# kv13arm/mujoco_rl_manipulate_unknown_objects

Measured on NVIDIA B200. Metric: env-steps/sec (acorn_env, 4096 envs/GPU), higher is better.
Workload: dtype f32

## Files before the change

mujoco_rl_manipulate_unknown_objects_b200/csrc/dev_model.cpp:

```cpp
#include <cstdlib>
#include <algorithm>
#include <cstring>
#include <stdexcept>

#include "model.h"

namespace grs {

void build_dev_model(const HostModel& h, DevModel& d, std::vector<float>& hv4, std::vector<int>& adj) {
  std::memset(&d, 0, sizeof d);
  if (h.nq != NQ || h.nv != NV || h.nu != NU)
    throw std::runtime_error("scene does not have the gripper-scene shape nq=14 nv=13 nu=7 (got nq=" + std::to_string(h.nq) + " nv=" + std::to_string(h.nv) +
                             " nu=" + std::to_string(h.nu) + ")");
  if (h.nbody > MAXB || h.njnt > MAXJ || h.ngeom > MAXG || h.npair > MAXPAIR || h.ncam > MAXCAM)
    throw std::runtime_error("scene exceeds the compiled-in limits (bodies/joints/geoms/pairs/cameras)");
  if (h.body_ee < 0 || h.body_object < 0 || h.finger1[0] < 0 || h.finger1[1] < 0 || h.finger2[0] < 0 || h.finger2[1] < 0)
    throw std::runtime_error("scene lacks one of the named bodies ee / object / {left,right}_inner_{knuckle,finger}");
  d.nbody = h.nbody; d.njnt = h.njnt; d.ngeom = h.ngeom; d.npair = h.npair; d.iterations = h.iterations; d.ncam = h.ncam;
  d.timestep = (float)h.timestep; d.impratio = (float)h.impratio; d.meaninertia = (float)h.meaninertia;
  d.solver_scale = (float)(1.0 / (h.meaninertia * std::max(1, h.nv)));
  d.gap_skip = getenv("GRS_GAP_SKIP") ? atoi(getenv("GRS_GAP_SKIP")) : 1;
  d.newton_noise = getenv("GRS_NEWTON_NOISE") ? (float)atof(getenv("GRS_NEWTON_NOISE")) : 3.6e-7f;
  for (int k = 0; k < 3; k++) d.gravity[k] = (float)h.gravity[k];
  d.xfrc_ee_z = (float)(-(0.438 * h.gravity[2]));
  std::vector<int> depth(h.nbody, 0);
  int maxd = 0;
  for (int b = 1; b < h.nbody; b++) { depth[b] = depth[h.body_parentid[b]] + 1; maxd = std::max(maxd, depth[b]); }
  if (maxd + 1 > MAXLEVEL) throw std::runtime_error("kinematic tree is deeper than the compiled-in limit");
  d.nlevel = maxd + 1;
  int n = 0;
  for (int lv = 0; lv <= maxd; lv++) {
    d.level_start[lv] = n;
    for (int b = 0; b < h.nbody; b++) if (depth[b] == lv) d.level_body[n++] = b;
  }
  for (int lv = maxd + 1; lv <= MAXLEVEL; lv++) d.level_start[lv] = n;
  for (int b = 0; b < h.nbody; b++) {
    d.body_parent[b] = h.body_parentid[b]; d.body_root[b] = h.body_rootid[b];
    d.body_jntadr[b] = h.body_jntadr[b] < 0 ? 0 : h.body_jntadr[b]; d.body_jntnum[b] = h.body_jntnum[b];
    d.body_dofadr[b] = h.body_dofadr[b] < 0 ? 0 : h.body_dofadr[b]; d.body_dofnum[b] = h.body_dofnum[b];
    for (int k = 0; k < 3; k++) { d.body_pos[b][k] = (float)h.body_pos[3 * b + k]; d.body_ipos[b][k] = (float)h.body_ipos[3 * b + k]; d.body_inertia[b][k] = (float)h.body_inertia[3 * b + k]; }
    for (int k = 0; k < 4; k++) { d.body_quat[b][k] = (float)h.body_quat[4 * b + k]; d.body_iquat[b][k] = (float)h.body_iquat[4 * b + k]; }
    d.body_mass[b] = (float)h.body_mass[b];
    d.body_invweight0[b][0] = (float)h.body_invweight0[2 * b]; d.body_invweight0[b][1] = (float)h.body_invweight0[2 * b + 1];
    unsigned mask = 0;
    for (int c = 0; c < h.nbody; c++) {
      int a = c;
      while (a != b && a > 0) a = h.body_parentid[a];
      if (a == b) mask |= 1u << c;
    }
    d.body_subtree_mask[b] = mask;
    unsigned dm = 0;
    for (int a = b; a > 0; a = h.body_parentid[a])
      for (int k = 0; k < h.body_dofnum[a]; k++) dm |= 1u << (h.body_dofadr[a] + k);
    d.body_dofmask[b] = dm;
  }
  for (int j = 0; j < h.njnt; j++) {
    d.jnt_type[j] = h.jnt_type[j]; d.jnt_body[j] = h.jnt_bodyid[j]; d.jnt_qposadr[j] = h.jnt_qposadr[j];
    d.jnt_dofadr[j] = h.jnt_dofadr[j]; d.jnt_limited[j] = h.jnt_limited[j];
    for (int k = 0; k < 3; k++) { d.jnt_pos[j][k] = (float)h.jnt_pos[3 * j + k]; d.jnt_axis[j][k] = (float)h.jnt_axis[3 * j + k]; }
    d.jnt_range[j][0] = (float)h.jnt_range[2 * j]; d.jnt_range[j][1] = (float)h.jnt_range[2 * j + 1];
    d.jnt_qpos0[j] = (float)h.qpos0[h.jnt_qposadr[j]];
  }
  for (int k = 0; k < 2; k++) d.jnt_solref[k] = (float)h.jnt_solref[k];
  for (int k = 0; k < 5; k++) d.jnt_solimp[k] = (float)h.jnt_solimp[k];
  for (int k = 0; k < NQ; k++) d.qpos0[k] = (float)h.qpos0[k];
  for (int i = 0; i < NV; i++) {
    d.dof_body[i] = h.dof_bodyid[i]; d.dof_jnt[i] = h.dof_jntid[i];
    unsigned am = 0;
    for (int a = i; a >= 0; a = h.dof_parentid[a]) am |= 1u << a;
    d.dof_ancmask[i] = am;
    d.dof_armature[i] = (float)h.dof_armature[i]; d.dof_damping[i] = (float)h.dof_damping[i]; d.dof_invweight0[i] = (float)h.dof_invweight0[i];
  }
  for (int i = 0; i < NV; i++) {
    unsigned blk = i < 7 ? 0x7fu : (0x3fu << 7);
    if (d.dof_ancmask[i] & ~blk) throw std::runtime_error("dof tree layout is not 7 gripper dofs followed by 6 free-object dofs");
  }
  hv4.clear(); adj.clear();
  for (int g = 0; g < h.ngeom; g++) {
    d.geom_type[g] = h.geom_type[g]; d.geom_body[g] = h.geom_bodyid[g];
    for (int k = 0; k < 3; k++) d.geom_pos[g][k] = (float)h.geom_pos[3 * g + k];
    for (int k = 0; k < 4; k++) d.geom_quat[g][k] = (float)h.geom_quat[4 * g + k];
    d.geom_rbound[g] = (float)h.geom_rbound[g];
    for (int k = 0; k < 3; k++) d.geom_size[g][k] = (float)h.geom_size[3 * g + k];
    if (h.geom_meshid[g] >= 0) {
      const HostMesh& ms = h.meshes[h.geom_meshid[g]];
      int nvert = (int)ms.hull_verts.size() / 3;
      d.geom_hvadr[g] = (int)hv4.size() / 4; d.geom_hvnum[g] = nvert;
      for (int i = 0; i < nvert; i++) { for (int k = 0; k < 3; k++) hv4.push_back((float)ms.hull_verts[3 * i + k]); hv4.push_back(0.0f); }
      d.geom_adjadr[g] = (int)adj.size();
      adj.insert(adj.end(), ms.adjadr.begin(), ms.adjadr.end());
      adj.insert(adj.end(), ms.adj.begin(), ms.adj.end());
    }
  }
  d.nhv_total = (int)hv4.size() / 4;
  for (int p = 0; p < h.npair; p++) {
    int g1 = h.pair_geom1[p], g2 = h.pair_geom2[p];
    d.pair_g1[p] = g1; d.pair_g2[p] = g2;
    if (std::max(h.geom_condim[g1], h.geom_condim[g2]) != 4)
      throw std::runtime_error("only condim-4 contact pairs are supported (the reference scenes' default geom condim)");
    if (std::max(h.geom_gap[g1], h.geom_gap[g2]) != 0) throw std::runtime_error("geom gap is not supported");
    d.pair_margin[p] = (float)std::max(h.geom_margin[g1], h.geom_margin[g2]);
    for (int k = 0; k < 3; k++) d.pair_fric[p][k] = (float)std::max(h.geom_friction[3 * g1 + k], h.geom_friction[3 * g2 + k]);
    for (int k = 0; k < 2; k++) d.pair_solref[p][k] = (float)(0.5 * (h.geom_solref[2 * g1 + k] + h.geom_solref[2 * g2 + k]));
    for (int k = 0; k < 5; k++) d.pair_solimp[p][k] = (float)(0.5 * (h.geom_solimp[5 * g1 + k] + h.geom_solimp[5 * g2 + k]));
  }
  for (int u = 0; u < NU; u++) {
    d.act_dof[u] = h.act_dofid[u]; d.act_gear[u] = (float)h.act_gear[u];
    d.act_lo[u] = (float)std::max(-1e30, h.act_ctrlrange[2 * u]); d.act_hi[u] = (float)std::min(1e30, h.act_ctrlrange[2 * u + 1]);
  }
  d.body_ee = h.body_ee; d.body_object = h.body_object;
  for (int k = 0; k < 2; k++) { d.finger1[k] = h.finger1[k]; d.finger2[k] = h.finger2[k]; }
  for (int c = 0; c < h.ncam; c++) {
    d.cam_body[c] = h.cam_bodyid[c]; d.cam_mode[c] = h.cam_mode[c]; d.cam_target[c] = h.cam_target[c];
    for (int k = 0; k < 3; k++) d.cam_pos[c][k] = (float)h.cam_pos[3 * c + k];
    for (int k = 0; k < 4; k++) d.cam_quat[c][k] = (float)h.cam_quat[4 * c + k];
    d.cam_fovy[c] = (float)h.cam_fovy[c];
  }
}

}
```

mujoco_rl_manipulate_unknown_objects_b200/csrc/model.h:

```cpp
#pragma once
#include <array>
#include <string>
#include <vector>

namespace grs {

constexpr int NQ = 14, NV = 13, NU = 7;
constexpr int MAXB = 10, MAXJ = 8, MAXG = 8, MAXPAIR = 16, MAXMESH = 6, MAXLEVEL = 6;
constexpr int MAXCAM = 4, MAXLIGHT = 4;

enum GeomType { GEOM_PLANE = 0, GEOM_BOX = 6, GEOM_MESH = 7 };
enum JointType { JNT_FREE = 0, JNT_SLIDE = 2, JNT_HINGE = 3 };

struct HostMesh {
  std::string name;
  std::array<double, 3> pos{};
  std::array<double, 4> quat{1, 0, 0, 0};
  double volume = 0;
  std::array<double, 3> inertia_unit{};
  std::vector<double> hull_verts;
  std::vector<int> hull_faces;
  std::vector<int> adjadr, adj;
  std::vector<float> tri;
};

struct HostModel {
  int nbody = 0, njnt = 0, nq = 0, nv = 0, nu = 0, ngeom = 0, nmesh = 0, npair = 0, ncam = 0, nlight = 0;
  double timestep = 0.002, gravity[3] = {0, 0, -9.81}, impratio = 1, tolerance = 1e-8, znear = 0.01, zfar = 50;
  int iterations = 100, cone_elliptic = 0;
  std::vector<std::string> body_names, geom_names, jnt_names, cam_names;
  std::vector<int> body_parentid, body_weldid, body_jntadr, body_jntnum, body_dofadr, body_dofnum, body_rootid;
  std::vector<double> body_pos, body_quat, body_ipos, body_iquat, body_mass, body_inertia, body_invweight0;
  std::vector<int> jnt_type, jnt_bodyid, jnt_qposadr, jnt_dofadr, jnt_limited;
  std::vector<double> jnt_pos, jnt_axis, jnt_range, qpos0;
  double jnt_solref[2] = {0.02, 1}, jnt_solimp[5] = {0.9, 0.95, 0.001, 0.5, 2};
  std::vector<int> dof_bodyid, dof_jntid, dof_parentid;
  std::vector<double> dof_armature, dof_damping, dof_invweight0;
  std::vector<int> geom_type, geom_bodyid, geom_meshid, geom_condim;
  std::vector<double> geom_pos, geom_quat, geom_friction, geom_margin, geom_gap, geom_solref, geom_solimp,
      geom_rbound, geom_rgba, geom_size, geom_mass, geom_matprop;
  std::vector<HostMesh> meshes;
  std::vector<int> act_dofid;
  std::vector<double> act_gear, act_ctrlrange;
  std::vector<int> pair_geom1, pair_geom2;
  std::vector<int> cam_bodyid, cam_mode, cam_target;
  std::vector<double> cam_pos, cam_quat, cam_fovy;
  std::vector<int> light_bodyid, light_directional;
  std::vector<double> light_pos, light_dir, light_diffuse, light_ambient, light_specular;
  double meaninertia = 1, extent = 1, center[3] = {0, 0, 0};
  double tex_rgb1[3] = {0.1, 0.2, 0.3}, tex_rgb2[3] = {0.2, 0.3, 0.4}, texrepeat[2] = {1, 1};
  double sky_rgb1[3] = {0.3, 0.5, 0.7}, sky_rgb2[3] = {0, 0, 0};
  int body_ee = -1, body_object = -1, finger1[2] = {-1, -1}, finger2[2] = {-1, -1};
};

HostModel compile_mjcf(const std::string& xml_path);

struct DevModel {
  int nbody, njnt, ngeom, npair, nlevel, nhv_total, iterations, ncam;
  float timestep, impratio, meaninertia, solver_scale;
  int gap_skip;
  float newton_noise;
  float gravity[3], xfrc_ee_z;
  int level_start[MAXLEVEL + 1];
  int level_body[MAXB];
  int body_parent[MAXB], body_root[MAXB], body_jntadr[MAXB], body_jntnum[MAXB], body_dofadr[MAXB], body_dofnum[MAXB];
  unsigned body_subtree_mask[MAXB];
  unsigned body_dofmask[MAXB];
  float body_pos[MAXB][3], body_quat[MAXB][4], body_ipos[MAXB][3], body_iquat[MAXB][4];
  float body_mass[MAXB], body_inertia[MAXB][3], body_invweight0[MAXB][2];
  int jnt_type[MAXJ], jnt_body[MAXJ], jnt_qposadr[MAXJ], jnt_dofadr[MAXJ], jnt_limited[MAXJ];
  float jnt_pos[MAXJ][3], jnt_axis[MAXJ][3], jnt_range[MAXJ][2], jnt_qpos0[MAXJ];
  float jnt_solref[2], jnt_solimp[5], padj;
  float qpos0[NQ + 2];
  int dof_body[NV + 3], dof_jnt[NV + 3];
  unsigned dof_ancmask[NV + 3];
  float dof_armature[NV + 3], dof_damping[NV + 3], dof_invweight0[NV + 3];
  int geom_type[MAXG], geom_body[MAXG], geom_hvadr[MAXG], geom_hvnum[MAXG], geom_adjadr[MAXG];
  float geom_pos[MAXG][3], geom_quat[MAXG][4], geom_rbound[MAXG], geom_size[MAXG][3];
  int pair_g1[MAXPAIR], pair_g2[MAXPAIR];
  float pair_margin[MAXPAIR], pair_fric[MAXPAIR][3] , pair_solref[MAXPAIR][2], pair_solimp[MAXPAIR][5];
  int act_dof[NU + 1];
  float act_gear[NU + 1], act_lo[NU + 1], act_hi[NU + 1];
  int body_ee, body_object, finger1[2], finger2[2], pad2, pad3;
  int cam_body[MAXCAM], cam_mode[MAXCAM], cam_target[MAXCAM];
  float cam_pos[MAXCAM][3], cam_quat[MAXCAM][4], cam_fovy[MAXCAM];
};

void build_dev_model(const HostModel& h, DevModel& d, std::vector<float>& hull_verts4, std::vector<int>& hull_adj);

}
```

mujoco_rl_manipulate_unknown_objects_b200/csrc/sim_kernels.cuh:

```cuda
#pragma once
#include <cuda_runtime.h>
#include <stdint.h>

#include "model.h"

namespace grs {

constexpr int MAXCON = 12;
constexpr int MAXEFC = MAXCON * 4 + 7;
constexpr unsigned FULL = 0xffffffffu;
constexpr float MINVAL = 1e-15f;

struct __align__(16) WS {
  float qpos[16], qvel[16], ctrl[8], warm[16];
  float xpos[MAXB][3], xquat[MAXB][4], xmat[MAXB][9];
  float xanchor[MAXJ][3], xaxis[MAXJ][3];
  float gpos[MAXG][3], gmat[MAXG][9];
  float com[MAXB][3];
  float cdof[16][6];
  float M[NV * NV];
  int ncon, nefc, nlim, overflow, coupled, padi[3];
  float c_dist[MAXCON], c_pos[MAXCON][3], c_frame[MAXCON][9], c_mu[MAXCON], c_fric[MAXCON][3];
  int c_g1[MAXCON], c_g2[MAXCON], c_pair[MAXCON];
  float fsmooth[16], asmooth[16], qacc[16], Ma[16], grad[16], search[16], Mv[16], fcon[16], bias[16];
// ... 110 lines not shown
  for (int k = 0; k < NB; k++) {
    a[k] = 0.0f;
    if (k < nb) {
      if (is_row && k <= lr) a[k] = A[lane * NV + base + k];
      else if (is_rhs) a[k] = tmp[base + k];
    }
  }
#pragma unroll
  for (int j = 0; j < NB; j++) {
    if (is_row && lr >= j) A[lane * NV + base + j] = a[j];
    __syncwarp();
    const int cj = base + (j < nb ? j : 0);
    const float djj = A[cj * NV + cj];
    float rs = rsqrtf(fmaxf(djj, 1e-30f));
    rs = rs * (1.5f - 0.5f * djj * rs * rs);
    const float t = a[j] * rs * rs;
    a[j] *= rs;
#pragma unroll
    for (int k = j + 1; k < NB; k++) {
      const int rk = base + (k < nb ? k : 0);
      a[k] -= t * A[rk * NV + cj];
    }
  }
  __syncwarp();
  if (is_row) {
#pragma unroll
    for (int k = 0; k < NB; k++)
      if (k <= lr) A[lane * NV + base + k] = a[k];
  }
  if (is_rhs) {
#pragma unroll
    for (int k = 0; k < NB; k++)
      if (k < nb) tmp[base + k] = a[k];
  }
  __syncwarp();
  float y = is_row ? tmp[lane] : 0.0f;
#pragma unroll
  for (int j = NB - 1; j >= 0; j--) {
    const bool valid = j < nb;
    const int gj = base + (valid ? j : 0);
    const float ljj = A[gj * NV + gj];
    if (is_row && valid && lr == j) tmp[gj] = __fdividef(y, ljj);
    __syncwarp();
    const float xj = tmp[gj];
    if (is_row && valid) {
      if (lr == j) y = xj;
      else if (lr < j) y -= A[gj * NV + lane] * xj;
    }
  }
  __syncwarp();
  return y;
}

__device__ __noinline__ void kinematics(const DevModel& m, WS& w, int lane) {
  if (lane == 0) {
    for (int j = 0; j < m.njnt; j++)
      if (m.jnt_type[j] == JNT_FREE) quat_normalize(w.qpos + m.jnt_qposadr[j] + 3);
    w.xpos[0][0] = w.xpos[0][1] = w.xpos[0][2] = 0;
    w.xquat[0][0] = 1; w.xquat[0][1] = w.xquat[0][2] = w.xquat[0][3] = 0;
    quat2mat(w.xmat[0], w.xquat[0]);
  }
  __syncwarp();
  for (int lv = 1; lv < m.nlevel; lv++) {
    int idx = m.level_start[lv] + lane;
    if (idx < m.level_start[lv + 1]) {
      int b = m.level_body[idx], pid = m.body_parent[b];
      int jadr = m.body_jntadr[b], jnum = m.body_jntnum[b];
      float pos[3], quat[4];
      if (jnum == 1 && m.jnt_type[jadr] == JNT_FREE) {
        int qa = m.jnt_qposadr[jadr];
        for (int k = 0; k < 3; k++) pos[k] = w.qpos[qa + k];
        for (int k = 0; k < 4; k++) quat[k] = w.qpos[qa + 3 + k];
        for (int k = 0; k < 3; k++) { w.xanchor[jadr][k] = pos[k]; w.xaxis[jadr][k] = 0; }
      } else {
        float t[3];
        mulmat3vec(t, w.xmat[pid], m.body_pos[b]);
        for (int k = 0; k < 3; k++) pos[k] = w.xpos[pid][k] + t[k];
        quat_mul(quat, w.xquat[pid], m.body_quat[b]);
        for (int kj = 0; kj < jnum; kj++) {
          int j = jadr + kj;
          float anchor[3], axis[3];
          rot_vec_quat(t, m.jnt_pos[j], quat);
          for (int k = 0; k < 3; k++) anchor[k] = pos[k] + t[k];
          rot_vec_quat(axis, m.jnt_axis[j], quat);
          float q = w.qpos[m.jnt_qposadr[j]] - m.jnt_qpos0[j];
          if (m.jnt_type[j] == JNT_SLIDE) {
            for (int k = 0; k < 3; k++) pos[k] += axis[k] * q;
          } else {
            float s, c, ql[4];
            sincosf(0.5f * q, &s, &c);
            ql[0] = c; ql[1] = m.jnt_axis[j][0] * s; ql[2] = m.jnt_axis[j][1] * s; ql[3] = m.jnt_axis[j][2] * s;
            quat_mul(quat, quat, ql);
            rot_vec_quat(t, m.jnt_pos[j], quat);
            for (int k = 0; k < 3; k++) pos[k] = anchor[k] - t[k];
          }
          for (int k = 0; k < 3; k++) { w.xanchor[j][k] = anchor[k]; w.xaxis[j][k] = axis[k]; }
        }
      }
      quat_normalize(quat);
      for (int k = 0; k < 3; k++) w.xpos[b][k] = pos[k];
      for (int k = 0; k < 4; k++) w.xquat[b][k] = quat[k];
      quat2mat(w.xmat[b], quat);
    }
    __syncwarp();
  }
  if (lane < m.ngeom) {
    int g = lane, b = m.geom_body[g];
    float t[3], q[4], R[9];
    mulmat3vec(t, w.xmat[b], m.geom_pos[g]);
    quat_mul(q, w.xquat[b], m.geom_quat[g]);
    quat_normalize(q);
    quat2mat(R, q);
    float d2 = 0, r2 = 0;
    for (int k = 0; k < 3; k++) { const float np_ = w.xpos[b][k] + t[k], d = np_ - w.gpos[g][k]; d2 += d * d; w.gpos[g][k] = np_; }
    for (int k = 0; k < 9; k++) { const float d = R[k] - w.gmat[g][k]; r2 += d * d; w.gmat[g][k] = R[k]; }
    w.disp[g] = sqrtf(d2) + m.geom_rbound[g] * sqrtf(r2);
  }
  __syncwarp();
}

__device__ __noinline__ void com_pos_crb(const DevModel& m, WS& w, int lane) {
  const int nb = m.nbody;
  if (lane < nb) {
    int b = lane;
    float t[3], qi[4];
    mulmat3vec(t, w.xmat[b], m.body_ipos[b]);
    for (int k = 0; k < 3; k++) w.u.dyn.xipos[b][k] = w.xpos[b][k] + t[k];
    quat_mul(qi, w.xquat[b], m.body_iquat[b]);
    quat2mat(w.u.dyn.ximat[b], qi);
  }
  __syncwarp();
  if (lane < nb) {
    int r = m.body_root[lane];
    unsigned mask = m.body_subtree_mask[r];
    float s[3] = {0, 0, 0}, ms = 0;
    for (int b = 1; b < nb; b++)
      if ((mask >> b) & 1u) {
        float mb = m.body_mass[b];
        ms += mb;
        for (int k = 0; k < 3; k++) s[k] += mb * w.u.dyn.xipos[b][k];
      }
    if (ms < MINVAL) { for (int k = 0; k < 3; k++) w.com[lane][k] = w.u.dyn.xipos[r][k]; }
    else { float inv = 1.0f / ms; for (int k = 0; k < 3; k++) w.com[lane][k] = s[k] * inv; }
  }
  __syncwarp();
  if (lane < nb) {
    int b = lane;
    float* c = w.u.dyn.cinert[b];
    if (b == 0) { for (int k = 0; k < 10; k++) c[k] = 0; }
    else {
      const float* R = w.u.dyn.ximat[b];
      const float* I = m.body_inertia[b];
      float mb = m.body_mass[b], off[3];
      for (int k = 0; k < 3; k++) off[k] = w.u.dyn.xipos[b][k] - w.com[b][k];
      float dd = dot3(off, off);
      float M00 = R[0] * I[0] * R[0] + R[1] * I[1] * R[1] + R[2] * I[2] * R[2];
      float M11 = R[3] * I[0] * R[3] + R[4] * I[1] * R[4] + R[5] * I[2] * R[5];
      float M22 = R[6] * I[0] * R[6] + R[7] * I[1] * R[7] + R[8] * I[2] * R[8];
      float M01 = R[0] * I[0] * R[3] + R[1] * I[1] * R[4] + R[2] * I[2] * R[5];
      float M02 = R[0] * I[0] * R[6] + R[1] * I[1] * R[7] + R[2] * I[2] * R[8];
      float M12 = R[3] * I[0] * R[6] + R[4] * I[1] * R[7] + R[5] * I[2] * R[8];
      c[0] = M00 + mb * (dd - off[0] * off[0]);
      c[1] = M11 + mb * (dd - off[1] * off[1]);
      c[2] = M22 + mb * (dd - off[2] * off[2]);
      c[3] = M01 - mb * off[0] * off[1];
      c[4] = M02 - mb * off[0] * off[2];
      c[5] = M12 - mb * off[1] * off[2];
      c[6] = mb * off[0]; c[7] = mb * off[1]; c[8] = mb * off[2];
      c[9] = mb;
    }
  }
  if (lane < NV) {
    int i = lane, j = m.dof_jnt[i], b = m.dof_body[i], da = m.jnt_dofadr[j];
    float* c = w.cdof[i];
    int type = m.jnt_type[j];
    if (type == JNT_FREE) {
      int k = i - da;
      if (k < 3) { c[0] = c[1] = c[2] = 0; c[3] = k == 0; c[4] = k == 1; c[5] = k == 2; }
      else {
        k -= 3;
        float ax[3] = {w.xmat[b][k], w.xmat[b][3 + k], w.xmat[b][6 + k]}, off[3];
        for (int q = 0; q < 3; q++) off[q] = w.com[b][q] - w.xpos[b][q];
        c[0] = ax[0]; c[1] = ax[1]; c[2] = ax[2];
        cross3(c + 3, ax, off);
      }
    } else if (type == JNT_SLIDE) {
      c[0] = c[1] = c[2] = 0;
      for (int q = 0; q < 3; q++) c[3 + q] = w.xaxis[j][q];
    } else {
      float off[3], ax[3];
      for (int q = 0; q < 3; q++) { off[q] = w.com[b][q] - w.xanchor[j][q]; ax[q] = w.xaxis[j][q]; c[q] = ax[q]; }
      cross3(c + 3, ax, off);
    }
  }
  __syncwarp();
  if (lane < nb) {
    int b = lane;
    unsigned mask = m.body_subtree_mask[b];
    float acc[10];
    for (int k = 0; k < 10; k++) acc[k] = 0;
    if (b > 0)
      for (int bb = b; bb < nb; bb++)
        if ((mask >> bb) & 1u)
          for (int k = 0; k < 10; k++) acc[k] += w.u.dyn.cinert[bb][k];
    for (int k = 0; k < 10; k++) w.u.dyn.crb[b][k] = acc[k];
  }
  __syncwarp();
  float buf[6];
  if (lane < NV) mul_inert_vec(buf, w.u.dyn.crb[m.dof_body[lane]], w.cdof[lane]);
  float(*fb)[6] = w.u.dyn.cdofdot;
  if (lane < NV) for (int k = 0; k < 6; k++) fb[lane][k] = buf[k];
  __syncwarp();
  for (int e = lane; e < NV * NV; e += 32) {
    int i = e / NV, j = e - i * NV;
    int hi = i > j ? i : j, lo = i > j ? j : i;
    float v = 0;
    if ((m.dof_ancmask[hi] >> lo) & 1u) v = dot6(w.cdof[lo], fb[hi]);
    if (i == j) v += m.dof_armature[i];
    w.M[e] = v;
  }
  __syncwarp();
}

#define SUPV(k) (w.sup[k])
#define SUPV1(k) (w.sup[k] + 3)
#define SUPV2(k) (w.sup[k] + 6)

__device__ __forceinline__ unsigned sortable_key(float x) {
  const unsigned k = __float_as_uint(x + 0.0f);
  return (k & 0x80000000u) ? ~k : (k | 0x80000000u);
}
__device__ __noinline__ int support_geom(const DevModel& m, const WS& w, const float4* __restrict__ hv, int g, const float* dir, float* out, int lane) {
  const float* R = w.gmat[g];
  float l[3];
  mulmat3Tvec(l, R, dir);
  const float4* v = hv + m.geom_hvadr[g];
  const int n = m.geom_hvnum[g];
  float best = -3.0e38f;
  int bi = 0;
#pragma unroll 2
  for (int i = lane; i < n; i += 32) {
    float4 p = v[i];
    float s = fmaf(p.z, l[2], fmaf(p.y, l[1], p.x * l[0]));
    if (s > best) { best = s; bi = i; }
  }
  const unsigned key = sortable_key(best);
  const unsigned kmax = __reduce_max_sync(FULL, key);
  bi = (int)__reduce_min_sync(FULL, key == kmax ? (unsigned)bi : 0xffffffffu);
  float4 p = v[bi];
  float pv[3] = {p.x, p.y, p.z}, t[3];
  mulmat3vec(t, R, pv);
  out[0] = w.gpos[g][0] + t[0]; out[1] = w.gpos[g][1] + t[1]; out[2] = w.gpos[g][2] + t[2];
  return bi;
}
__device__ __noinline__ void support_md(const DevModel& m, WS& w, const float4* hv, int g1, int g2, float margin, const float* dir, int slot, int lane) {
  float n[3] = {dir[0], dir[1], dir[2]}, nd[3];
  normalize3(n);
  nd[0] = -n[0]; nd[1] = -n[1]; nd[2] = -n[2];
  const float *R1 = w.gmat[g1], *R2 = w.gmat[g2];
  float l1[3], l2[3];
  mulmat3Tvec(l1, R1, n);
  mulmat3Tvec(l2, R2, nd);
  const float4 *va = hv + m.geom_hvadr[g1], *vb = hv + m.geom_hvadr[g2];
  const int na = m.geom_hvnum[g1], nb = m.geom_hvnum[g2], nmax = max(na, nb);
  float besta = -3.0e38f, bestb = -3.0e38f;
  int ia = 0, ib = 0;
#pragma unroll 2
  for (int i = lane; i < nmax; i += 32) {
    if (i < na) {
      const float4 p = va[i];
// ... 244 lines not shown
      for (int k = 0; k < 3; k++) dif[k] = v[k] - w.gpos[g1][k];
      float dist = dot3(dif, n);
      if (dist > margin) continue;
      for (int k = 0; k < 3; k++) pos[k] = v[k] - 0.5f * dist * n[k];
      add_contact(m, w, p, dist, pos, n, lane);
      const int* ga = adj + m.geom_adjadr[g2];
      int nvert = m.geom_hvnum[g2];
      int e0 = __ldg(ga + vi), e1 = __ldg(ga + vi + 1), cnt = 1;
      const float4* hvg = hv + m.geom_hvadr[g2];
      for (int e = e0; e < e1 && cnt < 3; e++) {
        int nb = __ldg(ga + nvert + 1 + e);
        float4 q = hvg[nb];
        float qv[3] = {q.x, q.y, q.z}, t[3];
        mulmat3vec(t, w.gmat[g2], qv);
        for (int k = 0; k < 3; k++) { v[k] = w.gpos[g2][k] + t[k]; dif[k] = v[k] - w.gpos[g1][k]; }
        dist = dot3(dif, n);
        if (dist > margin) continue;
        for (int k = 0; k < 3; k++) pos[k] = v[k] - 0.5f * dist * n[k];
        add_contact(m, w, p, dist, pos, n, lane);
        cnt++;
      }
    } else {
      float depth, dir[3], pos[3];
      float ca[3] = {w.sep[p][0], w.sep[p][1], w.sep[p][2]};
      if (ca[0] != 0.0f || ca[1] != 0.0f || ca[2] != 0.0f) {
        support_md(m, w, hv, g1, g2, margin, ca, 4, lane);
        const float sd = dot3(SUPV(4), ca);
        if (sd < 0) {
          __syncwarp();
          if (lane == 0) w.gapb[p] = -sd - 2e-6f;
          __syncwarp();
          continue;
        }
      }
      bool hit = mpr_penetration(m, w, hv, g1, g2, margin, &depth, dir, pos, lane);
      __syncwarp();
      if (lane < 3) w.sep[p][lane] = hit ? 0.0f : dir[lane];
      if (lane == 3) w.gapb[p] = 0.0f;
      __syncwarp();
      if (!hit) continue;
      add_contact(m, w, p, margin - depth, pos, dir, lane);
    }
  }
  __syncwarp();
}

__device__ __forceinline__ void forward_position(const DevModel& m, WS& w, const float4* hv, const int* adj, int lane) {
  kinematics(m, w, lane);
  com_pos_crb(m, w, lane);
  collision(m, w, hv, adj, lane);
}

__device__ __noinline__ void smooth_forces(const DevModel& m, WS& w, int lane, bool actuation, float xfrc_z) {
  const int nb = m.nbody;
  if (lane == 0) for (int k = 0; k < 6; k++) { w.u.dyn.cvel[0][k] = 0; w.u.dyn.cfrc[0][k] = 0; }
  if (lane == 0) { float* a = w.u.dyn.crb[0]; a[0] = a[1] = a[2] = 0; a[3] = -m.gravity[0]; a[4] = -m.gravity[1]; a[5] = -m.gravity[2]; }
  __syncwarp();
  for (int lv = 1; lv < m.nlevel; lv++) {
    int idx = m.level_start[lv] + lane;
    if (idx < m.level_start[lv + 1]) {
      int b = m.level_body[idx], pid = m.body_parent[b];
      float cvel[6], cacc[6];
      for (int k = 0; k < 6; k++) { cvel[k] = w.u.dyn.cvel[pid][k]; cacc[k] = w.u.dyn.crb[pid][k]; }
      for (int kj = 0; kj < m.body_jntnum[b]; kj++) {
        int j = m.body_jntadr[b] + kj, a = m.jnt_dofadr[j];
        if (m.jnt_type[j] == JNT_FREE) {
          for (int i = 0; i < 3; i++) {
            for (int k = 0; k < 6; k++) w.u.dyn.cdofdot[a + i][k] = 0;
            float qv = w.qvel[a + i];
            for (int k = 0; k < 6; k++) cvel[k] += w.cdof[a + i][k] * qv;
          }
          float dd[3][6];
          for (int i = 0; i < 3; i++) cross_motion(dd[i], cvel, w.cdof[a + 3 + i]);
          for (int i = 0; i < 3; i++) {
            float qv = w.qvel[a + 3 + i];
            for (int k = 0; k < 6; k++) { w.u.dyn.cdofdot[a + 3 + i][k] = dd[i][k]; cvel[k] += w.cdof[a + 3 + i][k] * qv; cacc[k] += dd[i][k] * qv; }
          }
        } else {
          float dd[6], qv = w.qvel[a];
          cross_motion(dd, cvel, w.cdof[a]);
          for (int k = 0; k < 6; k++) { w.u.dyn.cdofdot[a][k] = dd[k]; cvel[k] += w.cdof[a][k] * qv; cacc[k] += dd[k] * qv; }
        }
      }
      float t1[6], t2[6], f[6];
      mul_inert_vec(t1, w.u.dyn.cinert[b], cacc);
      mul_inert_vec(t2, w.u.dyn.cinert[b], cvel);
      cross_force(f, cvel, t2);
      for (int k = 0; k < 6; k++) { w.u.dyn.cvel[b][k] = cvel[k]; w.u.dyn.crb[b][k] = cacc[k]; w.u.dyn.cfrc[b][k] = f[k] + t1[k]; }
    }
    __syncwarp();
  }
  float bias = 0;
  if (lane < NV) {
    int b = m.dof_body[lane];
    unsigned mask = m.body_subtree_mask[b];
    float acc[6] = {0, 0, 0, 0, 0, 0};
    for (int bb = b; bb < nb; bb++)
      if ((mask >> bb) & 1u)
        for (int k = 0; k < 6; k++) acc[k] += w.u.dyn.cfrc[bb][k];
    bias = dot6(w.cdof[lane], acc);
  }
  float f = 0;
  if (lane < NV) {
    f = -m.dof_damping[lane] * w.qvel[lane] - bias;
    if (actuation)
      for (int u = 0; u < NU; u++)
        if (m.act_dof[u] == lane) f += m.act_gear[u] * fminf(fmaxf(w.ctrl[u], m.act_lo[u]), m.act_hi[u]);
    if (xfrc_z != 0.0f && ((m.body_dofmask[m.body_ee] >> lane) & 1u)) {
      float off[3], t[3];
      for (int k = 0; k < 3; k++) off[k] = w.u.dyn.xipos[m.body_ee][k] - w.com[m.body_ee][k];
      cross3(t, w.cdof[lane], off);
      f += (w.cdof[lane][5] + t[2]) * xfrc_z;
    }
    w.bias[lane] = bias;
    w.fsmooth[lane] = f;
  }
  __syncwarp();
  for (int e = lane; e < NV * NV; e += 32) w.u.dyn.L[e] = w.M[e];
  __syncwarp();
  float a = chol_factor_solve<true>(w.u.dyn.L, w.cho, f, lane);
  if (lane < NV) w.asmooth[lane] = a;
  __syncwarp();
}

__device__ __noinline__ float get_impedance(const float* solimp, float pos, float margin) {
  if (solimp[0] == solimp[1] || solimp[2] <= MINVAL) return 0.5f * (solimp[0] + solimp[1]);
  float x = fabsf((pos - margin) / solimp[2]);
  if (x >= 1) return solimp[1];
  if (x <= 0) return solimp[0];
  float y, p = solimp[4], mid = solimp[3];
  if (p == 1.0f) y = x;
  else if (p == 2.0f) y = x <= mid ? x * x / mid : 1 - (1 - x) * (1 - x) / (1 - mid);
  else y = x <= mid ? powf(x, p) / powf(mid, p - 1) : 1 - powf(1 - x, p) / powf(1 - mid, p - 1);
  return solimp[0] + y * (solimp[1] - solimp[0]);
}

__device__ __noinline__ void make_constraint(const DevModel& m, WS& w, int lane) {
  bool active = false;
  float dist = 0, sign = 0;
  if (lane < m.njnt && m.jnt_limited[lane] && m.jnt_type[lane] != JNT_FREE) {
    float value = w.qpos[m.jnt_qposadr[lane]];
    float dl = value - m.jnt_range[lane][0], du = m.jnt_range[lane][1] - value;
    if (dl < 0) { active = true; dist = dl; sign = 1; }
    else if (du < 0) { active = true; dist = du; sign = -1; }
  }
  unsigned bal = __ballot_sync(FULL, active);
  int nlim = __popc(bal);
  int ncon = w.ncon;
  int nefc = nlim + 4 * ncon;
  for (int e = lane; e < nefc * NV; e += 32) (&w.u.con.J[0][0])[e] = 0;
// ... 365 lines not shown
```

Before: 24.88 million.

## Specialize kinematic tree traversal to compile-time gripper topology

Replaces the runtime level tables, subtree masks, dof ancestry masks and joint-type dispatch with compile-time constants for the fixed gripper tree, checked on the host and by static asserts. Kinematics, CRB and smooth-force passes now unroll over known bodies and joints. Hinge sin/cos values are computed in parallel across lanes before the level loop instead of serially inside it. The aim is fewer model-memory loads, fewer branches and less serial latency, at the cost of rejecting any scene with a different topology.

```diff
diff --git a/mujoco_rl_manipulate_unknown_objects_b200/csrc/dev_model.cpp b/mujoco_rl_manipulate_unknown_objects_b200/csrc/dev_model.cpp
--- a/mujoco_rl_manipulate_unknown_objects_b200/csrc/dev_model.cpp
+++ b/mujoco_rl_manipulate_unknown_objects_b200/csrc/dev_model.cpp
@@ -6,6 +6,22 @@
 #include "model.h"
 
 namespace grs {
+
+static void check_tree(const HostModel& h) {
+  auto same = [](const std::vector<int>& v, const int* t, int n) { return (int)v.size() == n && std::equal(v.begin(), v.end(), t); };
+  const char* what = nullptr;
+  if (h.nbody != tree::NBODY || h.njnt != tree::NJNT) what = "body / joint count";
+  else if (!same(h.body_parentid, tree::body_parent, tree::NBODY)) what = "body_parentid";
+  else if (!same(h.body_rootid, tree::body_root, tree::NBODY)) what = "body_rootid";
+  else if (!same(h.body_jntadr, tree::body_jntadr, tree::NBODY) || !same(h.body_jntnum, tree::body_jntnum, tree::NBODY)) what = "body_jntadr / body_jntnum";
+  else if (!same(h.body_dofadr, tree::body_dofadr, tree::NBODY) || !same(h.body_dofnum, tree::body_dofnum, tree::NBODY)) what = "body_dofadr / body_dofnum";
+  else if (!same(h.jnt_type, tree::jnt_type, tree::NJNT) || !same(h.jnt_bodyid, tree::jnt_body, tree::NJNT)) what = "joint types / joint bodies";
+  else if (!same(h.jnt_qposadr, tree::jnt_qposadr, tree::NJNT) || !same(h.jnt_dofadr, tree::jnt_dofadr, tree::NJNT)) what = "jnt_qposadr / jnt_dofadr";
+  else if (!same(h.dof_bodyid, tree::dof_body, NV) || !same(h.dof_parentid, tree::dof_parent, NV)) what = "dof_bodyid / dof_parentid";
+  if (what)
+    throw std::runtime_error(std::string("scene's kinematic tree differs from the gripper tree the step kernel is written for (") + what +
+                             "): world, two camera mounts, ee with 3 slides + 2 hinges, base link, two hinged knuckles with a finger each, one free object");
+}
 
 void build_dev_model(const HostModel& h, DevModel& d, std::vector<float>& hv4, std::vector<int>& adj) {
   std::memset(&d, 0, sizeof d);
@@ -16,6 +32,7 @@
     throw std::runtime_error("scene exceeds the compiled-in limits (bodies/joints/geoms/pairs/cameras)");
   if (h.body_ee < 0 || h.body_object < 0 || h.finger1[0] < 0 || h.finger1[1] < 0 || h.finger2[0] < 0 || h.finger2[1] < 0)
     throw std::runtime_error("scene lacks one of the named bodies ee / object / {left,right}_inner_{knuckle,finger}");
+  check_tree(h);
   d.nbody = h.nbody; d.njnt = h.njnt; d.ngeom = h.ngeom; d.npair = h.npair; d.iterations = h.iterations; d.ncam = h.ncam;
   d.timestep = (float)h.timestep; d.impratio = (float)h.impratio; d.meaninertia = (float)h.meaninertia;
   d.solver_scale = (float)(1.0 / (h.meaninertia * std::max(1, h.nv)));
@@ -23,32 +40,13 @@
   d.newton_noise = getenv("GRS_NEWTON_NOISE") ? (float)atof(getenv("GRS_NEWTON_NOISE")) : 3.6e-7f;
   for (int k = 0; k < 3; k++) d.gravity[k] = (float)h.gravity[k];
   d.xfrc_ee_z = (float)(-(0.438 * h.gravity[2]));
-  std::vector<int> depth(h.nbody, 0);
-  int maxd = 0;
-  for (int b = 1; b < h.nbody; b++) { depth[b] = depth[h.body_parentid[b]] + 1; maxd = std::max(maxd, depth[b]); }
-  if (maxd + 1 > MAXLEVEL) throw std::runtime_error("kinematic tree is deeper than the compiled-in limit");
-  d.nlevel = maxd + 1;
-  int n = 0;
-  for (int lv = 0; lv <= maxd; lv++) {
-    d.level_start[lv] = n;
-    for (int b = 0; b < h.nbody; b++) if (depth[b] == lv) d.level_body[n++] = b;
-  }
-  for (int lv = maxd + 1; lv <= MAXLEVEL; lv++) d.level_start[lv] = n;
   for (int b = 0; b < h.nbody; b++) {
-    d.body_parent[b] = h.body_parentid[b]; d.body_root[b] = h.body_rootid[b];
-    d.body_jntadr[b] = h.body_jntadr[b] < 0 ? 0 : h.body_jntadr[b]; d.body_jntnum[b] = h.body_jntnum[b];
-    d.body_dofadr[b] = h.body_dofadr[b] < 0 ? 0 : h.body_dofadr[b]; d.body_dofnum[b] = h.body_dofnum[b];
+    d.body_root[b] = h.body_rootid[b];
+    d.body_jntadr[b] = h.body_jntadr[b] < 0 ? 0 : h.body_jntadr[b];
     for (int k = 0; k < 3; k++) { d.body_pos[b][k] = (float)h.body_pos[3 * b + k]; d.body_ipos[b][k] = (float)h.body_ipos[3 * b + k]; d.body_inertia[b][k] = (float)h.body_inertia[3 * b + k]; }
     for (int k = 0; k < 4; k++) { d.body_quat[b][k] = (float)h.body_quat[4 * b + k]; d.body_iquat[b][k] = (float)h.body_iquat[4 * b + k]; }
     d.body_mass[b] = (float)h.body_mass[b];
     d.body_invweight0[b][0] = (float)h.body_invweight0[2 * b]; d.body_invweight0[b][1] = (float)h.body_invweight0[2 * b + 1];
-    unsigned mask = 0;
-    for (int c = 0; c < h.nbody; c++) {
-      int a = c;
-      while (a != b && a > 0) a = h.body_parentid[a];
-      if (a == b) mask |= 1u << c;
-    }
-    d.body_subtree_mask[b] = mask;
     unsigned dm = 0;
     for (int a = b; a > 0; a = h.body_parentid[a])
       for (int k = 0; k < h.body_dofnum[a]; k++) dm |= 1u << (h.body_dofadr[a] + k);
@@ -65,15 +63,7 @@
   for (int k = 0; k < 5; k++) d.jnt_solimp[k] = (float)h.jnt_solimp[k];
   for (int k = 0; k < NQ; k++) d.qpos0[k] = (float)h.qpos0[k];
   for (int i = 0; i < NV; i++) {
-    d.dof_body[i] = h.dof_bodyid[i]; d.dof_jnt[i] = h.dof_jntid[i];
-    unsigned am = 0;
-    for (int a = i; a >= 0; a = h.dof_parentid[a]) am |= 1u << a;
-    d.dof_ancmask[i] = am;
     d.dof_armature[i] = (float)h.dof_armature[i]; d.dof_damping[i] = (float)h.dof_damping[i]; d.dof_invweight0[i] = (float)h.dof_invweight0[i];
-  }
-  for (int i = 0; i < NV; i++) {
-    unsigned blk = i < 7 ? 0x7fu : (0x3fu << 7);
-    if (d.dof_ancmask[i] & ~blk) throw std::runtime_error("dof tree layout is not 7 gripper dofs followed by 6 free-object dofs");
   }
   hv4.clear(); adj.clear();
   for (int g = 0; g < h.ngeom; g++) {
diff --git a/mujoco_rl_manipulate_unknown_objects_b200/csrc/model.h b/mujoco_rl_manipulate_unknown_objects_b200/csrc/model.h
--- a/mujoco_rl_manipulate_unknown_objects_b200/csrc/model.h
+++ b/mujoco_rl_manipulate_unknown_objects_b200/csrc/model.h
@@ -6,11 +6,42 @@
 namespace grs {
 
 constexpr int NQ = 14, NV = 13, NU = 7;
-constexpr int MAXB = 10, MAXJ = 8, MAXG = 8, MAXPAIR = 16, MAXMESH = 6, MAXLEVEL = 6;
+constexpr int MAXB = 10, MAXJ = 8, MAXG = 8, MAXPAIR = 16, MAXMESH = 6;
 constexpr int MAXCAM = 4, MAXLIGHT = 4;
 
 enum GeomType { GEOM_PLANE = 0, GEOM_BOX = 6, GEOM_MESH = 7 };
 enum JointType { JNT_FREE = 0, JNT_SLIDE = 2, JNT_HINGE = 3 };
+
+namespace tree {
+enum Body { WORLD = 0, CAM0 = 1, CAM1 = 2, EE = 3, BASE = 4, LKNUCKLE = 5, LFINGER = 6, RKNUCKLE = 7, RFINGER = 8, OBJECT = 9, NBODY = 10 };
+constexpr int NJNT = 8, JOBJECT = 7;
+constexpr int body_parent[NBODY] = {0, WORLD, WORLD, WORLD, EE, BASE, LKNUCKLE, BASE, RKNUCKLE, WORLD};
+constexpr int body_root[NBODY] = {WORLD, CAM0, CAM1, EE, EE, EE, EE, EE, EE, OBJECT};
+constexpr int body_jntadr[NBODY] = {-1, -1, -1, 0, -1, 5, -1, 6, -1, JOBJECT};
+constexpr int body_jntnum[NBODY] = {0, 0, 0, 5, 0, 1, 0, 1, 0, 1};
+constexpr int body_dofadr[NBODY] = {-1, -1, -1, 0, -1, 5, -1, 6, -1, 7};
+constexpr int body_dofnum[NBODY] = {0, 0, 0, 5, 0, 1, 0, 1, 0, 6};
+constexpr int jnt_type[NJNT] = {JNT_SLIDE, JNT_SLIDE, JNT_SLIDE, JNT_HINGE, JNT_HINGE, JNT_HINGE, JNT_HINGE, JNT_FREE};
+constexpr int jnt_body[NJNT] = {EE, EE, EE, EE, EE, LKNUCKLE, RKNUCKLE, OBJECT};
+constexpr int jnt_qposadr[NJNT] = {0, 1, 2, 3, 4, 5, 6, 7};
+constexpr int jnt_dofadr[NJNT] = {0, 1, 2, 3, 4, 5, 6, 7};
+constexpr int dof_body[NV] = {EE, EE, EE, EE, EE, LKNUCKLE, RKNUCKLE, OBJECT, OBJECT, OBJECT, OBJECT, OBJECT, OBJECT};
+constexpr int dof_parent[NV] = {-1, 0, 1, 2, 3, 4, 4, -1, 7, 8, 9, 10, 11};
+constexpr unsigned subtree_mask(int b) {
+  unsigned mask = 0;
+  for (int c = 0; c < NBODY; c++) {
+    int a = c;
+    while (a != b && a > 0) a = body_parent[a];
+    if (a == b) mask |= 1u << c;
+  }
+  return mask;
+}
+constexpr bool dof_is_ancestor(int hi, int lo) {
+  for (int a = hi; a >= 0; a = dof_parent[a])
+    if (a == lo) return true;
+  return false;
+}
+}
 
 struct HostMesh {
   std::string name;
@@ -56,15 +87,12 @@
 HostModel compile_mjcf(const std::string& xml_path);
 
 struct DevModel {
-  int nbody, njnt, ngeom, npair, nlevel, nhv_total, iterations, ncam;
+  int nbody, njnt, ngeom, npair, nhv_total, iterations, ncam;
   float timestep, impratio, meaninertia, solver_scale;
   int gap_skip;
   float newton_noise;
   float gravity[3], xfrc_ee_z;
-  int level_start[MAXLEVEL + 1];
-  int level_body[MAXB];
-  int body_parent[MAXB], body_root[MAXB], body_jntadr[MAXB], body_jntnum[MAXB], body_dofadr[MAXB], body_dofnum[MAXB];
-  unsigned body_subtree_mask[MAXB];
+  int body_root[MAXB], body_jntadr[MAXB];
   unsigned body_dofmask[MAXB];
   float body_pos[MAXB][3], body_quat[MAXB][4], body_ipos[MAXB][3], body_iquat[MAXB][4];
   float body_mass[MAXB], body_inertia[MAXB][3], body_invweight0[MAXB][2];
@@ -72,8 +100,6 @@
   float jnt_pos[MAXJ][3], jnt_axis[MAXJ][3], jnt_range[MAXJ][2], jnt_qpos0[MAXJ];
   float jnt_solref[2], jnt_solimp[5], padj;
   float qpos0[NQ + 2];
-  int dof_body[NV + 3], dof_jnt[NV + 3];
-  unsigned dof_ancmask[NV + 3];
   float dof_armature[NV + 3], dof_damping[NV + 3], dof_invweight0[NV + 3];
   int geom_type[MAXG], geom_body[MAXG], geom_hvadr[MAXG], geom_hvnum[MAXG], geom_adjadr[MAXG];
   float geom_pos[MAXG][3], geom_quat[MAXG][4], geom_rbound[MAXG], geom_size[MAXG][3];
diff --git a/mujoco_rl_manipulate_unknown_objects_b200/csrc/sim_kernels.cuh b/mujoco_rl_manipulate_unknown_objects_b200/csrc/sim_kernels.cuh
--- a/mujoco_rl_manipulate_unknown_objects_b200/csrc/sim_kernels.cuh
+++ b/mujoco_rl_manipulate_unknown_objects_b200/csrc/sim_kernels.cuh
@@ -186,49 +186,109 @@
   return y;
 }
 
+static_assert(tree::jnt_qposadr[tree::JOBJECT] == 7 && tree::jnt_dofadr[tree::JOBJECT] == 7, "free joint at qpos 7 / dof 7");
+static_assert(tree::jnt_qposadr[6] == 6 && tree::jnt_dofadr[6] == 6, "hinges and slides: qpos address = dof address = joint id");
+static_assert(tree::jnt_type[0] == JNT_SLIDE && tree::jnt_type[1] == JNT_SLIDE && tree::jnt_type[2] == JNT_SLIDE && tree::jnt_type[3] == JNT_HINGE && tree::jnt_type[4] == JNT_HINGE && tree::jnt_type[5] == JNT_HINGE &&
+              tree::jnt_type[6] == JNT_HINGE, "joint types as kinematics writes them out");
+
+constexpr unsigned long long pack_subtrees(int first, int n) {
+  unsigned long long p = 0;
+  for (int i = 0; i < n; i++) p |= (unsigned long long)tree::subtree_mask(first + i) << (10 * i);
+  return p;
+}
+constexpr unsigned long long SUBTREE_LO = pack_subtrees(0, 6), SUBTREE_HI = pack_subtrees(6, tree::NBODY - 6);
+__host__ __device__ constexpr unsigned subtree_of(int b) {
+  return (unsigned)((b < 6 ? SUBTREE_LO >> (10 * b) : SUBTREE_HI >> (10 * (b - 6))) & 0x3ffu);
+}
+struct DepthSlot { int b, pid; bool on; };
+__host__ __device__ constexpr DepthSlot depth_slot(int d, int lane) {
+  return d == 1 ? DepthSlot{lane < 3 ? lane + 1 : tree::OBJECT, tree::WORLD, lane < 4}
+       : d == 2 ? DepthSlot{tree::BASE, tree::EE, lane == 0}
+       : DepthSlot{(d == 3 ? tree::LKNUCKLE : tree::LFINGER) + 2 * lane, d == 3 ? tree::BASE : tree::LFINGER + 2 * lane - 1, lane < 2};
+}
+constexpr int NDEPTH = 4;
+__host__ __device__ constexpr int jnt_first(int b) { return b == tree::EE ? 0 : b == tree::LKNUCKLE ? 5 : 6; }
+__host__ __device__ constexpr int jnt_count(int b) { return b == tree::EE ? 5 : b == tree::LKNUCKLE || b == tree::RKNUCKLE ? 1 : 0; }
+__host__ __device__ constexpr int root_of(int b) { return b < tree::EE ? b : b < tree::OBJECT ? tree::EE : tree::OBJECT; }
+__host__ __device__ constexpr int dof_body_of(int i) { return i < 5 ? tree::EE : i == 5 ? tree::LKNUCKLE : i == 6 ? tree::RKNUCKLE : tree::OBJECT; }
+__host__ __device__ constexpr bool dof_anc(int hi, int lo) { return hi < 7 ? (lo <= 4 || lo == hi) : lo >= 7; }
+constexpr bool lane_maps_match_tree() {
+  for (int b = 0; b < tree::NBODY; b++)
+    if (subtree_of(b) != tree::subtree_mask(b) || (subtree_of(b) & ((1u << b) - 1u)) || root_of(b) != tree::body_root[b]) return false;
+  int depth[tree::NBODY] = {0};
+  for (int d = 1; d <= NDEPTH; d++)
+    for (int lane = 0; lane < 32; lane++) {
+      const DepthSlot t = depth_slot(d, lane);
+      if (!t.on) continue;
+      if (depth[t.b] || t.pid != tree::body_parent[t.b] || depth[t.pid] != d - 1) return false;
+      depth[t.b] = d;
+      if (t.b != tree::OBJECT && (jnt_count(t.b) != tree::body_jntnum[t.b] || (jnt_count(t.b) && jnt_first(t.b) != tree::body_jntadr[t.b]))) return false;
+    }
+  for (int b = 1; b < tree::NBODY; b++)
+    if (!depth[b]) return false;
+  for (int i = 0; i < NV; i++) {
+    if (dof_body_of(i) != tree::dof_body[i]) return false;
+    for (int j = 0; j <= i; j++)
+      if (dof_anc(i, j) != tree::dof_is_ancestor(i, j)) return false;
+  }
+  return true;
+}
+static_assert(lane_maps_match_tree(), "lane maps disagree with the tree tables of model.h");
+
 __device__ __noinline__ void kinematics(const DevModel& m, WS& w, int lane) {
+  using namespace tree;
+  constexpr int QF = jnt_qposadr[JOBJECT];
   if (lane == 0) {
-    for (int j = 0; j < m.njnt; j++)
-      if (m.jnt_type[j] == JNT_FREE) quat_normalize(w.qpos + m.jnt_qposadr[j] + 3);
+    quat_normalize(w.qpos + QF + 3);
     w.xpos[0][0] = w.xpos[0][1] = w.xpos[0][2] = 0;
     w.xquat[0][0] = 1; w.xquat[0][1] = w.xquat[0][2] = w.xquat[0][3] = 0;
     quat2mat(w.xmat[0], w.xquat[0]);
   }
-  __syncwarp();
-  for (int lv = 1; lv < m.nlevel; lv++) {
-    int idx = m.level_start[lv] + lane;
-    if (idx < m.level_start[lv + 1]) {
-      int b = m.level_body[idx], pid = m.body_parent[b];
-      int jadr = m.body_jntadr[b], jnum = m.body_jntnum[b];
+  float* hsc = &w.u.dyn.cfrc[0][0];
+  if (lane >= 3 && lane < 7) {
+    float s, c;
+    sincosf(0.5f * (w.qpos[lane] - m.jnt_qpos0[lane]), &s, &c);
+    hsc[2 * (lane - 3)] = s; hsc[2 * (lane - 3) + 1] = c;
+  }
+  __syncwarp();
+#pragma unroll 1
+  for (int d = 1; d <= NDEPTH; d++) {
+    const DepthSlot t = depth_slot(d, lane);
+    if (t.on) {
+      const int b = t.b, pid = t.pid;
       float pos[3], quat[4];
-      if (jnum == 1 && m.jnt_type[jadr] == JNT_FREE) {
-        int qa = m.jnt_qposadr[jadr];
-        for (int k = 0; k < 3; k++) pos[k] = w.qpos[qa + k];
-        for (int k = 0; k < 4; k++) quat[k] = w.qpos[qa + 3 + k];
-        for (int k = 0; k < 3; k++) { w.xanchor[jadr][k] = pos[k]; w.xaxis[jadr][k] = 0; }
+      if (b == OBJECT) {
+        for (int k = 0; k < 3; k++) pos[k] = w.qpos[QF + k];
+        for (int k = 0; k < 4; k++) quat[k] = w.qpos[QF + 3 + k];
+        for (int k = 0; k < 3; k++) { w.xanchor[JOBJECT][k] = pos[k]; w.xaxis[JOBJECT][k] = 0; }
       } else {
         float t[3];
         mulmat3vec(t, w.xmat[pid], m.body_pos[b]);
         for (int k = 0; k < 3; k++) pos[k] = w.xpos[pid][k] + t[k];
         quat_mul(quat, w.xquat[pid], m.body_quat[b]);
-        for (int kj = 0; kj < jnum; kj++) {
-          int j = jadr + kj;
+        auto joint = [&](int j, bool slide) {
           float anchor[3], axis[3];
           rot_vec_quat(t, m.jnt_pos[j], quat);
           for (int k = 0; k < 3; k++) anchor[k] = pos[k] + t[k];
           rot_vec_quat(axis, m.jnt_axis[j], quat);
-          float q = w.qpos[m.jnt_qposadr[j]] - m.jnt_qpos0[j];
-          if (m.jnt_type[j] == JNT_SLIDE) {
+          float q = w.qpos[j] - m.jnt_qpos0[j];
+          if (slide) {
             for (int k = 0; k < 3; k++) pos[k] += axis[k] * q;
           } else {
-            float s, c, ql[4];
-            sincosf(0.5f * q, &s, &c);
+            const float s = hsc[2 * (j - 3)], c = hsc[2 * (j - 3) + 1];
+            float ql[4];
             ql[0] = c; ql[1] = m.jnt_axis[j][0] * s; ql[2] = m.jnt_axis[j][1] * s; ql[3] = m.jnt_axis[j][2] * s;
             quat_mul(quat, quat, ql);
             rot_vec_quat(t, m.jnt_pos[j], quat);
             for (int k = 0; k < 3; k++) pos[k] = anchor[k] - t[k];
           }
           for (int k = 0; k < 3; k++) { w.xanchor[j][k] = anchor[k]; w.xaxis[j][k] = axis[k]; }
+        };
+        if (b == EE) {
+#pragma unroll
+          for (int j = 0; j < 5; j++) joint(j, j < 3);
+        } else if (jnt_count(b)) {
+          joint(jnt_first(b), false);
         }
       }
       quat_normalize(quat);
@@ -254,8 +314,8 @@
 }
 
 __device__ __noinline__ void com_pos_crb(const DevModel& m, WS& w, int lane) {
-  const int nb = m.nbody;
-  if (lane < nb) {
+  using namespace tree;
+  if (lane < NBODY) {
     int b = lane;
     float t[3], qi[4];
     mulmat3vec(t, w.xmat[b], m.body_ipos[b]);
@@ -264,11 +324,12 @@
     quat2mat(w.u.dyn.ximat[b], qi);
   }
   __syncwarp();
-  if (lane < nb) {
-    int r = m.body_root[lane];
-    unsigned mask = m.body_subtree_mask[r];
+  if (lane < NBODY) {
+    const int r = root_of(lane);
+    const unsigned mask = subtree_of(r);
     float s[3] = {0, 0, 0}, ms = 0;
-    for (int b = 1; b < nb; b++)
+#pragma unroll
+    for (int b = 1; b < NBODY; b++)
       if ((mask >> b) & 1u) {
         float mb = m.body_mass[b];
         ms += mb;
@@ -278,7 +339,7 @@
     else { float inv = 1.0f / ms; for (int k = 0; k < 3; k++) w.com[lane][k] = s[k] * inv; }
   }
   __syncwarp();
-  if (lane < nb) {
+  if (lane < NBODY) {
     int b = lane;
     float* c = w.u.dyn.cinert[b];
     if (b == 0) { for (int k = 0; k < 10; k++) c[k] = 0; }
@@ -305,51 +366,54 @@
     }
   }
   if (lane < NV) {
-    int i = lane, j = m.dof_jnt[i], b = m.dof_body[i], da = m.jnt_dofadr[j];
+    const int i = lane;
     float* c = w.cdof[i];
-    int type = m.jnt_type[j];
-    if (type == JNT_FREE) {
-      int k = i - da;
+    if (i >= 7) {
+      int k = i - 7;
       if (k < 3) { c[0] = c[1] = c[2] = 0; c[3] = k == 0; c[4] = k == 1; c[5] = k == 2; }
       else {
         k -= 3;
-        float ax[3] = {w.xmat[b][k], w.xmat[b][3 + k], w.xmat[b][6 + k]}, off[3];
-        for (int q = 0; q < 3; q++) off[q] = w.com[b][q] - w.xpos[b][q];
+        float ax[3] = {w.xmat[OBJECT][k], w.xmat[OBJECT][3 + k], w.xmat[OBJECT][6 + k]}, off[3];
+        for (int q = 0; q < 3; q++) off[q] = w.com[OBJECT][q] - w.xpos[OBJECT][q];
         c[0] = ax[0]; c[1] = ax[1]; c[2] = ax[2];
         cross3(c + 3, ax, off);
       }
-    } else if (type == JNT_SLIDE) {
+    } else if (i < 3) {
       c[0] = c[1] = c[2] = 0;
-      for (int q = 0; q < 3; q++) c[3 + q] = w.xaxis[j][q];
+      for (int q = 0; q < 3; q++) c[3 + q] = w.xaxis[i][q];
     } else {
+      const int b = dof_body_of(i);
       float off[3], ax[3];
-      for (int q = 0; q < 3; q++) { off[q] = w.com[b][q] - w.xanchor[j][q]; ax[q] = w.xaxis[j][q]; c[q] = ax[q]; }
+      for (int q = 0; q < 3; q++) { off[q] = w.com[b][q] - w.xanchor[i][q]; ax[q] = w.xaxis[i][q]; c[q] = ax[q]; }
       cross3(c + 3, ax, off);
     }
   }
   __syncwarp();
-  if (lane < nb) {
+  if (lane < NBODY) {
     int b = lane;
-    unsigned mask = m.body_subtree_mask[b];
+    const unsigned mask = b > 0 ? subtree_of(b) : 0u;
     float acc[10];
     for (int k = 0; k < 10; k++) acc[k] = 0;
-    if (b > 0)
-      for (int bb = b; bb < nb; bb++)
-        if ((mask >> bb) & 1u)
-          for (int k = 0; k < 10; k++) acc[k] += w.u.dyn.cinert[bb][k];
+#pragma unroll
+    for (int bb = 1; bb < NBODY; bb++)
+      if ((mask >> bb) & 1u)
+        for (int k = 0; k < 10; k++) acc[k] += w.u.dyn.cinert[bb][k];
     for (int k = 0; k < 10; k++) w.u.dyn.crb[b][k] = acc[k];
   }
   __syncwarp();
   float buf[6];
-  if (lane < NV) mul_inert_vec(buf, w.u.dyn.crb[m.dof_body[lane]], w.cdof[lane]);
+  if (lane < NV) mul_inert_vec(buf, w.u.dyn.crb[dof_body_of(lane)], w.cdof[lane]);
   float(*fb)[6] = w.u.dyn.cdofdot;
   if (lane < NV) for (int k = 0; k < 6; k++) fb[lane][k] = buf[k];
   __syncwarp();
-  for (int e = lane; e < NV * NV; e += 32) {
+#pragma unroll
+  for (int it = 0; it < (NV * NV + 31) / 32; it++) {
+    const int e = lane + 32 * it;
+    if (e >= NV * NV) break;
     int i = e / NV, j = e - i * NV;
     int hi = i > j ? i : j, lo = i > j ? j : i;
     float v = 0;
-    if ((m.dof_ancmask[hi] >> lo) & 1u) v = dot6(w.cdof[lo], fb[hi]);
+    if (dof_anc(hi, lo)) v = dot6(w.cdof[lo], fb[hi]);
     if (i == j) v += m.dof_armature[i];
     w.M[e] = v;
   }
@@ -700,34 +764,41 @@
 }
 
 __device__ __noinline__ void smooth_forces(const DevModel& m, WS& w, int lane, bool actuation, float xfrc_z) {
-  const int nb = m.nbody;
+  using namespace tree;
   if (lane == 0) for (int k = 0; k < 6; k++) { w.u.dyn.cvel[0][k] = 0; w.u.dyn.cfrc[0][k] = 0; }
   if (lane == 0) { float* a = w.u.dyn.crb[0]; a[0] = a[1] = a[2] = 0; a[3] = -m.gravity[0]; a[4] = -m.gravity[1]; a[5] = -m.gravity[2]; }
   __syncwarp();
-  for (int lv = 1; lv < m.nlevel; lv++) {
-    int idx = m.level_start[lv] + lane;
-    if (idx < m.level_start[lv + 1]) {
-      int b = m.level_body[idx], pid = m.body_parent[b];
+#pragma unroll 1
+  for (int d = 1; d <= NDEPTH; d++) {
+    const DepthSlot t = depth_slot(d, lane);
+    if (t.on) {
+      const int b = t.b, pid = t.pid;
       float cvel[6], cacc[6];
       for (int k = 0; k < 6; k++) { cvel[k] = w.u.dyn.cvel[pid][k]; cacc[k] = w.u.dyn.crb[pid][k]; }
-      for (int kj = 0; kj < m.body_jntnum[b]; kj++) {
-        int j = m.body_jntadr[b] + kj, a = m.jnt_dofadr[j];
-        if (m.jnt_type[j] == JNT_FREE) {
-          for (int i = 0; i < 3; i++) {
-            for (int k = 0; k < 6; k++) w.u.dyn.cdofdot[a + i][k] = 0;
-            float qv = w.qvel[a + i];
-            for (int k = 0; k < 6; k++) cvel[k] += w.cdof[a + i][k] * qv;
-          }
-          float dd[3][6];
-          for (int i = 0; i < 3; i++) cross_motion(dd[i], cvel, w.cdof[a + 3 + i]);
-          for (int i = 0; i < 3; i++) {
-            float qv = w.qvel[a + 3 + i];
-            for (int k = 0; k < 6; k++) { w.u.dyn.cdofdot[a + 3 + i][k] = dd[i][k]; cvel[k] += w.cdof[a + 3 + i][k] * qv; cacc[k] += dd[i][k] * qv; }
-          }
-        } else {
+      if (b == OBJECT) {
+        constexpr int a = jnt_dofadr[JOBJECT];
+        for (int i = 0; i < 3; i++) {
+          for (int k = 0; k < 6; k++) w.u.dyn.cdofdot[a + i][k] = 0;
+          float qv = w.qvel[a + i];
+          for (int k = 0; k < 6; k++) cvel[k] += w.cdof[a + i][k] * qv;
+        }
+        float dd[3][6];
+        for (int i = 0; i < 3; i++) cross_motion(dd[i], cvel, w.cdof[a + 3 + i]);
+        for (int i = 0; i < 3; i++) {
+          float qv = w.qvel[a + 3 + i];
+          for (int k = 0; k < 6; k++) { w.u.dyn.cdofdot[a + 3 + i][k] = dd[i][k]; cvel[k] += w.cdof[a + 3 + i][k] * qv; cacc[k] += dd[i][k] * qv; }
+        }
+      } else {
+        auto dof = [&](int a) {
           float dd[6], qv = w.qvel[a];
           cross_motion(dd, cvel, w.cdof[a]);
           for (int k = 0; k < 6; k++) { w.u.dyn.cdofdot[a][k] = dd[k]; cvel[k] += w.cdof[a][k] * qv; cacc[k] += dd[k] * qv; }
+        };
+        if (b == EE) {
+#pragma unroll
+          for (int a = 0; a < 5; a++) dof(a);
+        } else if (jnt_count(b)) {
+          dof(jnt_first(b));
         }
       }
       float t1[6], t2[6], f[6];
@@ -740,10 +811,10 @@
   }
   float bias = 0;
   if (lane < NV) {
-    int b = m.dof_body[lane];
-    unsigned mask = m.body_subtree_mask[b];
+    const unsigned mask = subtree_of(dof_body_of(lane));
     float acc[6] = {0, 0, 0, 0, 0, 0};
-    for (int bb = b; bb < nb; bb++)
+#pragma unroll
+    for (int bb = EE; bb < NBODY; bb++)
       if ((mask >> bb) & 1u)
         for (int k = 0; k < 6; k++) acc[k] += w.u.dyn.cfrc[bb][k];
     bias = dot6(w.cdof[lane], acc);
```

Result: slower. 24.53 million (median of 6 runs) (-1.4%).
